# Xinglab/abPOA

Measured on AMD Instinct MI355X. Metric: read-sets/sec (consensus bit-exact) + DP Gcells/sec (roofline.dp_gcells_per_s), higher is better.
Workload: dtype int16

## Files before the change

### abpoa_amd/csrc/diag.h

```cpp
#pragma once
#include <stdint.h>

#if defined(__HIPCC__)
#define DIAG_HD __host__ __device__
#else
#define DIAG_HD
#endif

namespace abpoa_hip {

constexpr int DBG_NO_FAST_LOOPS = 64;
constexpr int DBG_KEEP_ROW_SLOTS = 128;
constexpr int DBG_WALK_REPORT = 256;
constexpr int DBG_WALK_GIVES_UP = 512;
constexpr int DBG_ONE_WAVE_BACKTRACK = 1024;
constexpr int DBG_CXX_TIGHT_LOOP = 2048;
constexpr int ABL_NO_ARENA_STORE = 1;
constexpr int ABL_FAST_NO_RING_STORE = 2,     ABL_GEN_FAKE_ARGMAX = 2;
constexpr int ABL_FAST_NO_ARGMAX = 4,         ABL_GEN_LITERAL_F_SCAN = 4;
constexpr int ABL_FAST_NO_F_CLOSED_FORM = 8,  ABL_GEN_NO_CHUNKS = 8;
constexpr int ABL_FAST_NO_GATHER = 16,        ABL_GEN_FAKE_GATHER = 16;
constexpr int ABL_FAST_NO_SLOW_F = 32,        ABL_GEN_NO_QUERY_PROFILE = 32;
constexpr int DBG_ABLATION_BITS = 63;
struct DbgBit { int value; const char *what; };
constexpr DbgBit DBG_BITS[] = {
    {DBG_ABLATION_BITS, "timing ablations of the row loops (1 .. 32: only in a `make prof` library, results wrong on purpose)"},
    {DBG_NO_FAST_LOOPS, "no fast row loops"}, {DBG_KEEP_ROW_SLOTS, "the tails keep the row loop's AlnOut.seg"}, {DBG_WALK_REPORT, "walk report in AlnOut.seg"},
    {DBG_WALK_GIVES_UP, "the direction-word walk gives up (NEED_SCORES)"}, {DBG_ONE_WAVE_BACKTRACK, "one wavefront per backtrack"},
    {DBG_CXX_TIGHT_LOOP, "the compiler's tight loop"},
};

#ifdef ABPOA_HIP_PROFILE
#define FSTAMP(I) { asm volatile("s_waitcnt lgkmcnt(0)" ::: "memory"); long long t_ = (long long)__builtin_amdgcn_s_memtime(); fseg[I] += t_ - fseg_last; fseg_last = t_; }
#else
#define FSTAMP(I)
#endif
#ifdef ABPOA_HIP_ASM_CENSUS
#define CENSUS_SLOT(I) ((I) == CEN_ONE_PRED ? CEN_CXX_TIGHT : (I))
#else
#define CENSUS_SLOT(I) (I)
#endif
#ifdef ABPOA_HIP_ROW_CENSUS
#define CENSUS_T0() const long long cen_t0 = (long long)__builtin_amdgcn_s_memtime();
#define CENSUS(I) { fseg[CENSUS_SLOT(I)] += census_pack(1, (long long)__builtin_amdgcn_s_memtime() - cen_t0); }
#else
#define CENSUS_T0()
#define CENSUS(I)
#endif
#ifdef ABPOA_HIP_WIDE_COUNTERS
#define WCOUNT(I) { fseg[I] += 1; }
#define WCOUNT_BODY(NCH) { fseg[WC_BODY] += wide_body_pack(1, 0, 0) + ((NCH) >= 9 ? (I16 ? wide_body_pack(0, 0, 1) : wide_body_pack(0, 1, 0)) : 0); }
#else
#define WCOUNT(I) {}
#define WCOUNT_BODY(NCH) {}
#endif
#ifdef ABPOA_HIP_ABLATE
#define ABL(BIT) (b.dbg & (BIT))
#else
#define ABL(BIT) false
#endif

constexpr int DIAG_SLOTS = 6;
// ... 27 lines not shown
```

### abpoa_amd/csrc/engine_options.cpp

```cpp
#include "engine_options.h"
#include "diag.h"
#include <atomic>
#include <cstdlib>
#include <cstring>
#include <mutex>
#include <string>

namespace abpoa_hip {
namespace {

struct Row { const char *name, *help; };
const std::string kDbgHelp = [] { std::string h = "D  bit mask handed to the kernels (DevBatch.dbg; diag.h):";
                                  for (const DbgBit &d : DBG_BITS) h += (&d == DBG_BITS ? " " : ", ") + std::to_string(d.value) + " " + d.what;
                                  return h; }();
const Row kTable[] = {
    {"ABPOA_GPU_DEVICES", "P  device ordinals abpoa_hip_msa_batch spreads its batches over: all | 0,1,... (default: the device of abpoa_hip_init)"},
    {"ABPOA_GPU_BATCHES_PER_DEVICE", "P  batches dealt per device queue [2]"},
    {"ABPOA_HIP_STRICT", "P  1: a call that would hand any read-set to the host driver fails with ABPOA_HIP_ESTRICT"},
    {"ABPOA_HIP_VERBOSE", "P  per-pass timings, residency and fallback reasons on stderr"},
    {"ABPOA_HIP_HOSTGRAPH", "T  1: the host driver for every job"},
    {"ABPOA_HIP_NO_DEVICE_STRAND", "T  1: -s jobs on the host driver"},
    {"ABPOA_HIP_NO_DEVICE_LOCAL", "T  1: local-mode jobs on the host driver"},
    {"ABPOA_HIP_NO_DEVICE_GENERAL", "T  1: general-kernel jobs on the host driver"},
    {"ABPOA_HIP_DEVICE_GENERAL", "T  1: the general kernel for every device-resident job"},
    {"ABPOA_HIP_LOCKSTEP", "T  1: one launch per phase and round also where the all-rounds kernel would run"},
    {"ABPOA_HIP_LATE_TAIL", "T  1: the helpers of the all-rounds kernel's backtrack start after the row loop, not under it"},
    {"ABPOA_HIP_NODIR", "T  1: score-record arenas instead of direction words"},
    {"ABPOA_HIP_DIR_WIDE", "T  1 / 0: direction words for wide-band alignments always / never (default: by residency and memory)"},
    {"ABPOA_HIP_NOFAST", "T  1: no fast row loops (general kernel)"},
    {"ABPOA_HIP_NOWIDE", "T  1: no wide row loop"},
    {"ABPOA_HIP_NOXL", "T  1: no long-read form of the wide row loop"},
    {"ABPOA_HIP_LOCAL_TEAM", "T  1 / 0: the four-wavefront local row loop always / never"},
    {"ABPOA_HIP_WIDE_LO", "T  smallest band half-width that takes the wide loop [40]"},
    {"ABPOA_HIP_RING_ROWS", "T  depth of the wide loop's score ring (4 | 8 | 16)"},
    {"ABPOA_HIP_EXTRA_ROUTE_MIN", "T  ragged sets with fewer extra columns keep the narrow loop"},
    {"ABPOA_HIP_NO_RAGGED_SPLIT", "T  1: read-sets with ragged read ends stay in the batch of the uniform ones (no all-rounds kernel for such a job)"},
    {"ABPOA_HIP_RAGGED_CONCURRENT", "T  1: the ragged batch of a mixed job runs on a second queue of the device beside the uniform batch (measured: see LOG.md)"},
    {"ABPOA_HIP_PASS_SETS", "T  read-sets per pass of the device-resident driver"},
    {"ABPOA_HIP_FIRST_PASS", "T  start the node-slot ladder (3x, 4.5x, 6x, 4096x) at its second / third / fourth pass: 1 / 2 / 3 (profiling runs of one step)"},
    {"ABPOA_HIP_NO_PASS_HINT", "T  1: always start the ladder at 3x"},
    {"ABPOA_HIP_GROUPS", "T  read-set groups of the host driver"},
    {"ABPOA_HIP_ARENA_PCT", "T  arena estimate in percent (overflow-retry tests)"},
    {"ABPOA_HIP_BT_BYTES", "T  LDS window of the tail kernel in bytes"},
    {"ABPOA_HIP_BT_WC", "T  columns per row of the tail's column-slice windows"},
    {"ABPOA_HIP_ORDER_LDS", "T  0: the row-order walk with global tables"},
    {"ABPOA_HIP_ORDER_CAP", "T  node capacity of the row-order walk's LDS tables"},
// ... 59 lines not shown
```

### abpoa_amd/csrc/rows_fast.h

```cpp
#pragma once
#include "dp_common.h"
#include "dir_plane.h"
#include "rows_tight_asm.h"
#include "wide_closed_forms.h"

namespace abpoa_hip {

template <typename T, int GAP> struct FastFmt { static constexpr int CW = GAP == 0 ? 2 : (GAP == 1 ? 4 : 8); };
static_assert(FastFmt<int, 0>::CW == record_values(ABPOA_HIP_LINEAR_GAP) && FastFmt<int, 1>::CW == record_values(ABPOA_HIP_AFFINE_GAP) && FastFmt<int, 2>::CW == record_values(ABPOA_HIP_CONVEX_GAP), "engine.h record_values");
template <typename T, int GAP> struct DirFmt {
    static constexpr int DB = GAP == 1 ? 2 : 4;
    static constexpr int UPV2 = Width<T>::PN * DB / 16;
    __device__ __host__ static constexpr int units(int nv) { return (nv * UPV2 + 1) >> 1; }
};
template <int GAP> __device__ __forceinline__ unsigned dir_word(unsigned kf, unsigned u1, unsigned u2, unsigned d1, unsigned d2) {
    static_assert(DIRA_DF1_SH - DIRA_UE1_SH == 3 && DIRC_UE2_SH - DIRC_UE1_SH == 3 && DIRC_DF2_SH - DIRC_DF1_SH == 3 && DIRC_DF1_SH - DIRC_UE1_SH == 8, "field layout of dir_plane.h");
    if (GAP == 1) return (((d1 << 3) | u1) << DIRA_UE1_SH) | kf;
    return (((((d2 << 3) | d1) << 8) | ((u2 << 3) | u1)) << DIRC_UE1_SH) | kf;
}
template <int GAP> __device__ __forceinline__ unsigned dir_pack(unsigned kM, unsigned kE1, unsigned kE2, unsigned u1, unsigned u2, unsigned d1, unsigned d2) {
    return dir_word<GAP>(GAP == 1 ? (kE1 << DIRA_KE1_SH) | kM : (((kE2 << 4) | kE1) << DIRC_KE1_SH) | kM, u1, u2, d1, d2);
}
__device__ __forceinline__ unsigned umin_(unsigned a, unsigned b) { return a < b ? a : b; }
template <typename T> __device__ __forceinline__ unsigned dir_literal(int Hm1, int Fm1, int F, int oe, int e) {
// ... 65 lines not shown
    int *fr = (int *)(lds_raw + ph_off + b.lds.fr_off);
    typedef __attribute__((address_space(3))) int lds_int_t;
    const int vslot = (int)(unsigned)(size_t)(lds_int_t *)fr + 4 * ((threadIdx.x & 63 & (RR - 1)) * (NPW * RCS) + 2);
    auto ring_at = [&](int slot_addr, int col_idx) __attribute__((always_inline)) { return (const int *)(lds_int_t *)(size_t)(unsigned)(slot_addr + 4 * col_idx); };
    int *s_mx = (int *)(lds_raw + (WIDEB ? b.lds.w_mx_off : b.lds.mx_off));
    auto qat = [&](int j) __attribute__((always_inline)) -> int {
        if constexpr (WIDEB) return ((int)s_query[j >> 1] >> ((j & 1) * 4)) & 15; else return (int)s_query[j];
    };
    const int infw = I16 ? (int)(((unsigned)inf & 0xffffu) | ((unsigned)inf << 16)) : inf;
    const int qlen_sn = qlen / PN;
    auto wr = [](int x) __attribute__((always_inline)) { return (int)(T)x; };

    const int idist = inj_dist<PN>(l);
    const int inj1 = idist >= 0 ? inf - idist * e1 : INT_MIN, inj2 = idist >= 0 ? inf - idist * e2 : INT_MIN;
    const int le1 = lane * e1, le2 = lane * e2;
    const int cf1 = oe1 - e1 + le1, cf2 = oe2 - e2 + le2;
    const long long lo_ll = (long long)(I16 ? INT16_MIN : INT32_MIN) + imax(oe1, oe2) + (long long)PN * imax(e1, e2);
    const int fast_lo = (int)lo_ll;
    const int kconst = I16 ? argmax_key16_const(PN, l, vvl) : 0;
    const int ktie = argmax_tie32(PN, l, vvl);

    { GLOBAL_AS const int32_t *g_mat = vgpr_ptr(b.mat); for (int i = lane; i < m * m1; i += 64) { const int bb = i / m1, qc = i - bb * m1; s_mx[i] = qc < m ? g_mat[bb * m + qc] : 0; } }
    for (int i = lane; i < RR * NPW * RCS; i += 64) { const int pl = (i / RCS) % NPW; fr[i] = (I16 && pl == 0) ? infw : ((EPACK && pl == 1) ? 0 : inf); }
    WG_SYNC();
    auto ring_put = [&](int slot, int x, int H, int E1, int E2) __attribute__((always_inline)) {
        int *q = fr + slot * (NPW * RCS) + 2 + x;
        if (I16) { q[0] = (int)(((unsigned)H & 0xffffu) | ((unsigned)E1 << 16)); if (GAP == 2) q[RCS] = E2; }
        else { q[0] = H; if (GAP != 0) q[RCS] = E1; if (GAP == 2) q[2 * RCS] = E2; }
    };

    const bool extend = sgpr(b.align_mode == ABPOA_HIP_EXTEND_MODE ? 1 : 0) != 0;
    int ex_best = inf, ex_i = 0, ex_j = 0, ex_rem = 0; bool zstop = false;
    const bool asm_tight_on = sgpr(!(b.dbg & DBG_CXX_TIGHT_LOOP) && RC == 128 && b.align_mode != ABPOA_HIP_EXTEND_MODE ? 1 : 0) != 0;
    int cur = 0, n_vec_lane = 0;
    const int cap_pn = (int)(d.plane_cap / PN > 0x7fffffffLL ? 0x7fffffffLL : d.plane_cap / PN);
    const int cap_turbo = cap_pn - (DIR ? dir_units(NV) + NV * CWR : NV * CW);
    const int remain_end = __builtin_amdgcn_readfirstlane(io.row_remain[gn - 1]);
    int vg_geo = 0, vg_mi = 0, vg_off = 0;
    int vg_vm = 0, rowmax = 0;
    {
        const int r = __builtin_amdgcn_readfirstlane(io.row_remain[0]) - remain_end - 1;
        const int dp_end0 = imin(qlen, imax(0, qlen - r) + w);
        const int end_sn0 = dp_end0 / PN, W0 = (end_sn0 + 1) * PN;
        if ((long long)W0 * CWR > d.plane_cap) { status = ABPOA_HIP_STATUS_OVERFLOW; cursor_out = 0; n_cells_out = 0; rows_done_out = 0; return; }
        const bool ring0 = W0 <= RC && !EPACK;
        T *H = io.planes;
        for (int i = lane; i < W0; i += 64) {
            int h, x1 = inf, x2 = inf, f1 = inf, f2 = inf;
            if (GAP == 0) h = wr(-e1 * i);
            else if (GAP == 1) { const int g = wr(-o1 - e1 * i); h = i == 0 ? 0 : g; x1 = i == 0 ? wr(-oe1) : inf; f1 = i == 0 ? inf : g; }
            else {
                const int g1 = wr(-o1 - e1 * i), g2 = wr(-o2 - e2 * i);
                h = i == 0 ? 0 : imax(g1, g2); x1 = i == 0 ? wr(-oe1) : inf; x2 = i == 0 ? wr(-oe2) : inf; f1 = i == 0 ? inf : g1; f2 = i == 0 ? inf : g2;
            }
            T *cellp = H + (long long)i * CWR;
            if constexpr (CPK) { cellp[0] = (T)h; cellp[1] = (T)(i == 0 ? (int)((unsigned)(h - x1) | ((unsigned)(h - x2) << 16)) : -1); }
            else if constexpr (CSP) { cellp[0] = (T)h; cellp[PL_E1] = (T)x1; if (GAP == 2) { cellp[PL_E2] = (T)x2; cellp[3] = (T)0; } }
            else if constexpr (GAP == 0) { cellp[0] = (T)h; cellp[1] = (T)0; }
            else {
                cellp[0] = (T)h; cellp[PL_E1] = (T)x1; cellp[PL_F1] = (T)f1;
                if (GAP == 2) { cellp[PL_E2] = (T)x2; cellp[PL_F2] = (T)f2; }
            }
            if (ring0) ring_put(0, i, h, x1, x2);
        }
        cur = (end_sn0 + 1) * CWR;
        if (lane == 0) { vg_geo = (end_sn0 << 12) | (ring0 ? GEO_RING : 0); vg_mi = 0; vg_off = DIR ? cur : 0; }
// ... 12 lines not shown
        MetaB q; const int np = a.pe - a.ps;
#pragma unroll
        for (int k = 0; k < NPM; ++k) q.p[k] = io.pred_row[a.ps + imin(k, imax(np - 1, 0))];
        return q;
    };
    MetaA a1 = load_a(0); MetaB b1 = load_b(a1); MetaA a2 = load_a(64);
    int tv_r1 = 0, tv_r2 = 0;
    int tv_meta = 0, tv_rterm = 0, tv_ps = 0, tv_p0 = 0, tv_p1 = 0, tv_p2 = 0, tv_p3 = 0;
    int tv_p4 = 0, tv_p5 = 0, tv_p6 = 0, tv_p7 = 0;
    int tv_tb = 0;
    auto switch_tile = [&](int t0) __attribute__((always_inline)) {
        const int myrow = t0 + lane, np = a1.pe - a1.ps;
        bool fastrow = np >= 1 && np <= 4 && myrow < gn - 1 && myrow >= 1;
#pragma unroll
        for (int k = 0; k < 4; ++k) { const int dk = myrow - b1.p[k]; fastrow = fastrow && dk >= 1 && dk < RR; }
        tv_meta = (a1.base & 0xff) | (imin(np, 255) << 8) | (fastrow ? (1 << 16) : 0);
        if (!WIDEB) {
            tv_meta |= ((fastrow && np <= 2 && RC <= 128) ? (1 << 17) : 0) | ((fastrow && np >= 3 && RC <= 128) ? (1 << 18) : 0);
            bool row8 = np >= 5 && np <= 8 && myrow < gn - 1 && myrow >= 1 && RC <= 128;
#pragma unroll
            for (int k = 0; k < NPM; ++k) { const int dk = myrow - b1.p[k]; row8 = row8 && dk >= 1 && dk < RR; }
            tv_meta |= row8 ? (1 << 20) : 0;
        }
        {
            bool widerow = np >= 1 && np <= 8 && myrow < gn - 1 && myrow >= 1;
#pragma unroll
            for (int k = 0; k < NPM; ++k) { const int dk = myrow - b1.p[k]; widerow = widerow && dk >= 1 && dk < 64; }
            tv_meta |= widerow ? (1 << 19) : 0;
        }
        if constexpr (DIR) {
            const bool sp = a1.sd >= RR;
            if (sp) { tv_meta |= 1 << 21; if (tv_meta & (1 << 17)) tv_meta = (tv_meta & ~(1 << 17)) | (1 << 22); }
        }
        tv_tb = ((myrow - b1.p[0]) & 0xff) | (((myrow - b1.p[1]) & 0xff) << 8) | (((a1.base & 0xff) * m1 * 4) << 16);
        tv_rterm = qlen - (a1.rem - remain_end - 1); tv_ps = a1.ps;
        tv_r1 = imin(gn, tv_rterm) - w; tv_r2 = tv_rterm + w;
        tv_p0 = b1.p[0]; tv_p1 = b1.p[1]; tv_p2 = b1.p[2]; tv_p3 = b1.p[3];
        tv_p4 = b1.p[4]; tv_p5 = b1.p[5]; tv_p6 = b1.p[6]; tv_p7 = b1.p[7];
        a1 = a2; b1 = load_b(a1); a2 = load_a(t0 + 128);
    };
    int qc_beg_sn = -1, qoff0 = 0, qoff1 = 0;
    auto geo_of = [&](int p, int row, int &geo, int &mi, int &off) __attribute__((always_inline)) {
        if (row - p < 64) { const int sl = p & 63; geo = __builtin_amdgcn_readlane(vg_geo, sl); mi = __builtin_amdgcn_readlane(vg_mi, sl); off = __builtin_amdgcn_readlane(vg_off, sl); }
        else {
            geo = __builtin_amdgcn_readfirstlane(gld_i32(io.g_bsn + p) | (gld_i32(io.g_esn + p) << 12)); mi = __builtin_amdgcn_readfirstlane(gld_i32(io.row_max_i + p));
            off = __builtin_amdgcn_readfirstlane((int)(uint32_t)(gld_i64(io.g_coff + p) / PN));
        }
    };
    int beg_sn = 0, end_sn = 0, off_pn = 0, max_pe = 0, rterm = 0, base = 0, np = 0;
    bool to_ring = false;
    unsigned am_key = 0; int am_val = INT_MIN, am_v = 0, am_isend = 0; bool am_any = false;

    auto set_band = [&](auto pin, int mn_mi, int mx_mi, int min_pb) __attribute__((always_inline)) {
        auto S = [](int x) __attribute__((always_inline)) { if constexpr (decltype(pin)::value) return sgpr(x); else return x; };
        const int left = S(imin(gn, mn_mi + 1)), right = S(decltype(pin)::value ? mx_mi + 1 : imax(0, mx_mi + 1));
        const int lo = S(imin(left, rterm) - w), hi = S(imax(right, rterm) + w);
        const int beg = S(imax(0, lo)), end = S(imin(qlen, hi));
        beg_sn = imax((int)((unsigned)beg / PN), min_pb); end_sn = (int)((unsigned)end / PN);
    };
    auto refresh_qc = [&]() __attribute__((always_inline)) {
        if (beg_sn != qc_beg_sn) {
            qc_beg_sn = beg_sn;
            const int c0 = beg_sn * PN + lane, c1 = c0 + 64;
            qoff0 = (c0 >= 1 && c0 <= qlen) ? qat(c0 - 1) : m; qoff1 = (c1 >= 1 && c1 <= qlen) ? qat(c1 - 1) : m;
        }
    };
// ... 1062 lines not shown
```

### abpoa_amd/csrc/rows_tight_asm.h

```cpp
#pragma once
#define TA_SDWA0 " dst_sel:DWORD dst_unused:UNUSED_PAD src0_sel:WORD_0 src1_sel:DWORD\n\t"
#define TA_SDWA_S1W0 " dst_sel:DWORD dst_unused:UNUSED_PAD src0_sel:DWORD src1_sel:WORD_0\n\t"
#define TA_SDWA_S1W1 " dst_sel:DWORD dst_unused:UNUSED_PAD src0_sel:DWORD src1_sel:WORD_1\n\t"
#define TA_SDWA_S0W1 " dst_sel:DWORD dst_unused:UNUSED_PAD src0_sel:WORD_1 src1_sel:DWORD\n\t"
#define TA_DPP(CTRL) " " CTRL " bank_mask:0xf\n\t"
#define vQA "v104"
#define vCOL "v105"
#define vX "v106"
#define vQ "v107"
#define vR0 "v108"
#define vR1 "v109"
#define vR01 "v[108:109]"
#define vKC "v110"
#define vH "v111"
#define vHSE "v112"
#define vAK "v113"
#define vS1 "v114"
#define vG "v115"
#define vF "v115"
#define vQD "v116"
#define vRO "v117"
#define vHO "v118"
#define vT2A "v119"
#define vEN "v120"
// ... 3 lines not shown
#define vD "v123"
#define vKF "v124"
#define vWD "v124"
#define vX1 "v125"
#define vB0 "v126"
#define vB1 "v127"
#define vB01 "v[126:127]"
#define vMV "v100"
#define vE1 "v101"
#define vMV2 "v102"
#define vE12 "v103"
#define vT "v106"
#define vP "v125"
#define vFS "v126"
#define vSH "v127"
#define vKM "v92"
#define vKE "v93"
#define vX2 "v94"
#define vX3 "v95"
#define vC0 "v96"
#define vC1 "v97"
#define vC01 "v[96:97]"
#define vD0 "v98"
#define vD1 "v99"
#define vD01 "v[98:99]"

#define TA_BAND_BEG                                                                                          \
    "s_min_i32 %[sA], %[sA], %[sRT]\n\t"  "s_max_i32 %[sA], %[sA], 0\n\t"       "s_lshr_b32 %[sA], %[sA], 4\n\t"
#define TA_BAND_END                                                                                          \
    "s_max_i32 %[sB], %[sB], %[sR2]\n\t"  "s_min_i32 %[sB], %[sB], %[qlen]\n\t" "s_lshr_b32 %[sESN], %[sB], 4\n\t"
#define TA_QCACHE(LBL)                                                                                       \
    "s_cmp_lg_u32 %[sBSN], %[qcb]\n\t"     "s_cbranch_scc1 L_ref" LBL "_%=\n\t"                              \
    "L_refd" LBL "_%=:\n\t"
#define TA_CHECKS(SLOWLBL)                                                                                   \
    "s_sub_i32 %[sNV1], %[sESN], %[sBSN]\n\t"                                                                \
    "s_cmp_gt_u32 %[sNV1], 3\n\t"          "s_cbranch_scc1 L_dec_%=\n\t"                                     \
    "s_cmp_gt_i32 %[sESN], %[sPE0]\n\t"    "s_cbranch_scc1 " SLOWLBL "_%=\n\t"
#define TA_RINGCHK                                                                                           \
    "s_bitcmp0_b32 %[sG0], 24\n\t"         "s_cbranch_scc1 L_dec_%=\n\t"
#define TA_SLOW_ENTRY(SLOWLBL)                                                                               \
    TA_ALIGN SLOWLBL "_%=:\n\t"                                                                                       \
    "s_add_i32 %[sA], %[sPE0], 1\n\t"      "s_cmp_lg_u32 %[sESN], %[sA]\n\t"      "s_cbranch_scc1 L_dec_%=\n\t" \
    "s_cmp_gt_u32 %[sBSN], %[sPE0]\n\t"    "s_cbranch_scc1 L_dec_%=\n\t"
#define TA_S_YES(x) x
#define TA_S_NO(x) ""
#define TA_REFRESH(LBL)                                                                                      \
    "L_ref" LBL "_%=:\n\t"                                                                                   \
    "s_mov_b32 %[qcb], %[sBSN]\n\t"        "s_lshl_b32 %[sA], %[sBSN], 4\n\t"     "s_add_i32 %[sA], %[sA], -1\n\t"      \
    "v_add_u32 " vX ", %[sA], %[lane]\n\t" "v_cmp_gt_u32 vcc, %[qlen], " vX "\n\t" "v_add_u32 " vQ ", %[qb], " vX "\n\t" \
    "ds_read_u8 " vQ ", " vQ "\n\t"                                                                          \
    "v_add_u32 " vX ", 64, " vX "\n\t"     "v_cmp_gt_u32_e64 %[msk], %[qlen], " vX "\n\t" "v_add_u32 " vG ", %[qb], " vX "\n\t" \
    "ds_read_u8 " vG ", " vG "\n\t"        "v_mov_b32 " vX ", %[m]\n\t"                                      \
    "s_waitcnt lgkmcnt(0)\n\t"                                                                               \
    "v_cndmask_b32 %[qoff0], " vX ", " vQ ", vcc\n\t"   "v_cndmask_b32_e64 %[qoff1], " vX ", " vG ", %[msk]\n\t"  \
    "v_lshl_add_u32 " vQA ", %[qoff0], 2, %[mxb]\n\t"                                                        \
    "s_branch L_refd" LBL "_%=\n\t"
#define TA_READS                                                                                             \
    "s_lshl_b32 %[sC0], %[sBSN], 4\n\t"    "v_add_u32 " vCOL ", %[sC0], %[lane]\n\t"                         \
    "s_ashr_i32 %[sA], %[sTB], 16\n\t"     "v_add_u32 " vX ", %[sA], " vQA "\n\t"    "ds_read_b32 " vQ ", " vX "\n\t"   \
    "s_lshl_b32 %[sA], %[sPB0], 4\n\t"     "v_xad_u32 " vX ", %[sA], -1, " vCOL "\n\t"  "v_med3_i32 " vX ", " vX ", -2, %[rc]\n\t" \
    "v_lshl_add_u32 " vX ", " vX ", 2, %[sSL0]\n\t"   "ds_read2_b32 " vR01 ", " vX " offset1:1\n\t"
#define TA_MASKS                                                                                             \
    "v_cmp_ge_u32_e64 %[inb], %[sNV1], %[vvl]\n\t"                                                               \
    "v_cmp_eq_u32 vcc, %[sNV1], %[vvl]\n\t"      "v_cndmask_b32 " vKC ", %[kN], %[kE], vcc\n\t"              \
    "v_cmp_ge_i32_e64 %[amok], %[qlen], " vCOL "\n\t"  "s_and_b64 %[amok], %[amok], %[inb]\n\t"
#define TA_SCAN                                                                                              \
    "v_add_u32 " vG ", " vH ", %[le1]\n\t"                                                                  \
    "v_lshl_add_u32 " vAK ", " vHSE ", 16, " vKC "\n\t"   "v_cndmask_b32_e64 " vAK ", 0, " vAK ", %[amok]\n\t" \
    "v_subrev_u32 " vS1 ", %[e1], " vH "\n\t"                                                               \
    "v_mov_b32_dpp " vS1 ", " vG " wave_shr:1 row_mask:0xf bank_mask:0xf\n\t"                                \
    "v_max_u32_dpp " vAK ", " vAK ", " vAK TA_DPP("row_shr:1 row_mask:0xf")                                  \
    "v_readlane_b32 %[sP0], %[vslot], %[row]\n\t"                                                            \
    "v_max_i32_dpp " vS1 ", " vS1 ", " vS1 TA_DPP("row_shr:1 row_mask:0xf")                                  \
    "v_max_u32_dpp " vAK ", " vAK ", " vAK TA_DPP("row_shr:2 row_mask:0xf")                                  \
    "s_lshl_b32 %[sM0], %[cur], 5\n\t"                                                                       \
    "v_max_i32_dpp " vS1 ", " vS1 ", " vS1 TA_DPP("row_shr:2 row_mask:0xf")                                  \
// ... 29 lines not shown
    TA_SLOW_STEP("3", "16", "row_shr:8")
#define TA_SLOW_F                                                                                            \
    "v_cmp_eq_u32 vcc, %[sNV1], %[vvl]\n\t"     "v_cndmask_b32 " vF ", " vF ", " vFS ", vcc\n\t"
#define TA_SLOW_LIT                                                                                          \
    "v_mov_b32_dpp " vP ", " vHO " wave_shr:1 row_mask:0xf bank_mask:0xf\n\t"                                \
    "v_mov_b32_dpp " vSH ", " vF " wave_shr:1 row_mask:0xf bank_mask:0xf\n\t"                                \
    "v_subrev_u32 " vP ", %[oe1], " vP "\n\t"   "v_bfe_i32 " vP ", " vP ", 0, 16\n\t"   "v_cmp_eq_i32_e64 %[msk], " vP ", " vF "\n\t" \
    "v_subrev_u32 " vSH ", %[e1], " vSH "\n\t"  "v_bfe_i32 " vSH ", " vSH ", 0, 16\n\t" "v_cmp_eq_i32 vcc, " vSH ", " vF "\n\t" \
    "v_cndmask_b32_e64 " vSH ", 3, 2, vcc\n\t"  "v_cndmask_b32_e64 " vSH ", " vSH ", 1, %[msk]\n\t"          \
    "v_cmp_le_u32 vcc, %[sNV1], %[vvl]\n\t"     "v_cndmask_b32 " vSH ", 0, " vSH ", vcc\n\t"
#define TA_HEF(EN_INSTR, S)                                                                                  \
    "v_sub_u32 " vF ", " vS1 ", %[cf1]\n\t"     "v_max_i32 " vF ", " vF ", %[inj1]\n\t"                      \
    S(TA_SLOW_F)                                                                                             \
    "v_max_i32 " vHO ", " vHSE ", " vF "\n\t"   "v_subrev_u32 " vT2A ", %[oe1], " vHO "\n\t"                 \
    EN_INSTR                                                                                                 \
    "v_max_i32 " vEN ", " vEN ", " vT2A "\n\t"                                                               \
    "v_cmp_lt_i32 vcc, " vHSE ", " vF "\n\t"    "v_cndmask_b32 " vE ", " vEN ", %[infv], vcc\n\t"            \
    "v_sub_u32 " vU ", " vEN ", " vT2A "\n\t"   "v_sub_u32 " vD ", " vHO ", " vF "\n\t"     "v_min_u32 " vD ", 7, " vD "\n\t" \
    "v_perm_b32 " vHE ", " vE ", " vHO ", %[perm]\n\t"                                                       \
    S(TA_SLOW_LIT)
#define TA_TAIL(S)                                                                                           \
    "v_lshl_or_b32 " vU ", " vD ", 3, " vU "\n\t"   "v_lshl_or_b32 " vWD ", " vU ", 8, " vKF "\n\t"           \
    S("v_lshl_or_b32 " vWD ", " vSH ", 14, " vWD "\n\t")                                                     \
    "global_store_short " vRO ", " vWD ", %[planes]\n\t"                                                     \
    "v_cndmask_b32_e64 " vHE ", %[infwv], " vHE ", %[inb]\n\t"                                                   \
    "ds_write2st64_b32 " vQD ", " vHE ", %[infwv] offset1:1\n\t"                                             \
    "v_readlane_b32 %[sA], " vAK ", 63\n\t"                                                                  \
    "s_bitset1_b32 %[sB], 24\n\t"                                                                            \
    "v_writelane_b32 %[geo], %[sB], m0\n\t"     "v_writelane_b32 %[off], %[cur], m0\n\t"                     \
    "s_and_b32 %[sM0], %[sA], 63\n\t"           "s_add_i32 %[sM0], %[sM0], %[sC0]\n\t"                       \
    "s_cmp_gt_u32 %[sA], %[infk]\n\t"           "s_cselect_b32 %[sA], %[sM0], -1\n\t"       \
    "v_writelane_b32 %[mi], %[sA], m0\n\t"                                                                   \
    "s_add_i32 %[cur], %[cur], %[sNV1]\n\t"     "s_add_i32 %[cur], %[cur], 1\n\t"                            \
    "s_add_i32 %[row], %[row], 1\n\t"           "s_cmp_lt_i32 %[row], %[rhi]\n\t"     "s_cbranch_scc1 L_row_%=\n\t"

#define TA_IF4_YES(x) x
#define TA_IF4_NO(x) ""
#define TA_FOLD(LANE, SL, PB, PE)                                                                            \
    "v_readlane_b32 %[sM1], %[mi], " LANE "\n\t"  "v_readlane_b32 %[sG1], %[geo], " LANE "\n\t"  "v_readlane_b32 " SL ", %[vslot], " LANE "\n\t" \
    "s_min_i32 %[sA], %[sA], %[sM1]\n\t"          "s_max_i32 %[sB], %[sB], %[sM1]\n\t"           "s_and_b32 %[sG0], %[sG0], %[sG1]\n\t" \
    "s_and_b32 " PB ", %[sG1], 0xfff\n\t"         "s_bfe_u32 " PE ", %[sG1], 0xc000c\n\t"
#define TA_READK(X, PAIR, SL, PB, PE)                                                                        \
    "s_lshl_b32 %[sA], " PB ", 4\n\t"             "v_subrev_u32 " X ", %[sA], " vCOL "\n\t"                  \
    "v_add_u32 " vT ", -1, " X "\n\t"             "v_med3_i32 " vT ", " vT ", -2, %[rc]\n\t"                 \
    "v_lshl_add_u32 " vT ", " vT ", 2, " SL "\n\t"  "ds_read2_b32 " PAIR ", " vT " offset1:1\n\t"            \
    "s_sub_i32 " PE ", " PE ", " PB "\n\t"        "s_lshl_b32 " PE ", " PE ", 4\n\t"             "s_add_i32 " PE ", " PE ", 16\n\t"
#define TA_MERGE(KIDX, W0, W1, X, PE)                                                                        \
    "v_max_i32_sdwa " vT ", " vMV ", sext(" W0 ")" TA_SDWA_S1W0                                              \
    "v_cmp_lt_i32 vcc, " vMV ", " vT "\n\t"                                                                  \
    "s_add_i32 %[sA], " PE ", 16\n\t"             "v_cmp_gt_u32_e64 %[msk], %[sA], " X "\n\t"    "s_and_b64 vcc, vcc, %[msk]\n\t" \
    "v_cndmask_b32_e64 " vKM ", " vKM ", " KIDX ", vcc\n\t"   "v_cndmask_b32_e64 " vMV ", " vMV ", " vT ", %[msk]\n\t" \
    "v_max_i32_sdwa " vT ", " vE1 ", sext(" W1 ")" TA_SDWA_S1W1                                              \
    "v_cmp_lt_i32 vcc, " vE1 ", " vT "\n\t"                                                                  \
    "v_cmp_gt_u32_e64 %[msk], " PE ", " X "\n\t"  "s_and_b64 vcc, vcc, %[msk]\n\t"                           \
    "v_cndmask_b32_e64 " vKE ", " vKE ", " KIDX ", vcc\n\t"   "v_cndmask_b32_e64 " vE1 ", " vE1 ", " vT ", %[msk]\n\t"
#define TA_MULTI_POST(IF4, S)                                                                                \
    TA_RINGCHK                                                                                               \
    TA_MASKS                                                                                                 \
    "v_mov_b32 " vKM ", 1\n\t"                    "v_mov_b32 " vKE ", 1\n\t"                                 \
    "s_waitcnt lgkmcnt(0)\n\t"                                                                               \
    "v_bfe_i32 " vMV ", " vR0 ", 0, 16\n\t"       "v_ashrrev_i32 " vE1 ", 16, " vR1 "\n\t"                   \
    TA_MERGE("2", vB0, vB1, vX1, "%[sPE1]")                                                                  \
    TA_MERGE("3", vC0, vC1, vX2, "%[sPE2]")                                                                  \
    IF4(TA_MERGE("4", vD0, vD1, vX3, "%[sPE3]"))                                                             \
    "v_add_u32 " vH ", " vMV ", " vQ "\n\t"                                                                  \
    "v_min_i32 " vT ", " vH ", " vE1 "\n\t"                                                                  \
    "v_cmp_gt_i32 vcc, %[fastlo], " vT "\n\t"     "s_and_b64 %[msk], %[inb], vcc\n\t"   "s_cbranch_scc1 L_x2_%=\n\t"  \
    "v_max_i32 " vHSE ", " vH ", " vE1 "\n\t"                                                                \
    TA_SCAN                                                                                                  \
    S(TA_SLOW_A)                                                                                             \
    TA_HEF("v_subrev_u32 " vEN ", %[e1], " vE1 "\n\t", S)                                                    \
    "v_cmp_eq_u32 vcc, " vH ", " vHO "\n\t"       "v_cndmask_b32 " vKF ", 0, " vKM ", vcc\n\t"               \
    "v_lshl_or_b32 " vKF ", " vKE ", 4, " vKF "\n\t"                                                         \
    TA_TAIL(S)                                                                                               \
    "s_branch L_end_%=\n\t"
#define TA_MULTI(IF4, LBL)                                                                                   \
    "s_mov_b32 %[sA], %[sM0]\n\t"                 "s_mov_b32 %[sB], %[sM0]\n\t"                              \
    "s_and_b32 %[sPB0], %[sG0], 0xfff\n\t"        "s_bfe_u32 %[sPE0], %[sG0], 0xc000c\n\t"                   \
    TA_FOLD("%[sP1]", "%[sSL1]", "%[sPB1]", "%[sPE1]")                                                       \
    TA_FOLD("%[sP2]", "%[sSL2]", "%[sPB2]", "%[sPE2]")                                                       \
    IF4(TA_FOLD("%[sP3]", "%[sSL3]", "%[sPB3]", "%[sPE3]"))                                                  \
    "s_add_i32 %[sA], %[sA], %[c1]\n\t"               "s_add_i32 %[sB], %[sB], %[c2]\n\t"                            \
    TA_BAND_BEG                                                                                              \
    "s_min_u32 %[sESN], %[sPB0], %[sPB1]\n\t"     "s_min_u32 %[sESN], %[sESN], %[sPB2]\n\t"   IF4("s_min_u32 %[sESN], %[sESN], %[sPB3]\n\t") \
    "s_max_u32 %[sBSN], %[sA], %[sESN]\n\t"                                                                  \
    TA_QCACHE(LBL)                                                                                           \
    TA_READS                                                                                                 \
    "s_max_u32 %[sPE0], %[sPE0], %[sPE1]\n\t"     "s_max_u32 %[sPE0], %[sPE0], %[sPE2]\n\t" IF4("s_max_u32 %[sPE0], %[sPE0], %[sPE3]\n\t") \
    TA_READK(vX1, vB01, "%[sSL1]", "%[sPB1]", "%[sPE1]")                                                     \
    TA_READK(vX2, vC01, "%[sSL2]", "%[sPB2]", "%[sPE2]")                                                     \
    IF4(TA_READK(vX3, vD01, "%[sSL3]", "%[sPB3]", "%[sPE3]"))                                                \
    TA_BAND_END                                                                                              \
    TA_CHECKS("L_s" LBL)                                                                                     \
    TA_MULTI_POST(IF4, TA_S_NO)                                                                              \
    TA_SLOW_ENTRY("L_s" LBL)                                                                                 \
    TA_MULTI_POST(IF4, TA_S_YES)

#define TA_ONE_POST(S)                                                                                       \
    TA_RINGCHK                                                                                               \
    TA_MASKS                                                                                                 \
    "s_waitcnt lgkmcnt(0)\n\t"                                                                               \
    "v_add_u32_sdwa " vH ", sext(" vR0 "), " vQ TA_SDWA0                                                     \
    "v_min_i32_sdwa " vT ", " vH ", sext(" vR1 ")" TA_SDWA_S1W1                                              \
    "v_cmp_gt_i32 vcc, %[fastlo], " vT "\n\t"   "s_and_b64 %[msk], %[inb], vcc\n\t"   "s_cbranch_scc1 L_x2_%=\n\t"  \
    "v_max_i32_sdwa " vHSE ", " vH ", sext(" vR1 ")" TA_SDWA_S1W1                                            \
    TA_SCAN                                                                                                  \
    S(TA_SLOW_A)                                                                                             \
    TA_HEF("v_sub_u32_sdwa " vEN ", sext(" vR1 "), %[e1]" TA_SDWA_S0W1, S)                                   \
    "v_cmp_eq_u32 vcc, " vH ", " vHO "\n\t"     "v_cndmask_b32_e64 " vKF ", 16, 17, vcc\n\t"                 \
    TA_TAIL(S)                                                                                               \
    "s_branch L_end_%=\n\t"
#define TA_TWO_POST(S)                                                                                       \
    TA_RINGCHK                                                                                               \
    TA_MASKS                                                                                                 \
    "s_waitcnt lgkmcnt(0)\n\t"                                                                               \
    "v_bfe_i32 " vMV ", " vR0 ", 0, 16\n\t"     "v_ashrrev_i32 " vE1 ", 16, " vR1 "\n\t"                     \
    "v_max_i32_sdwa " vT ", " vMV ", sext(" vB0 ")" TA_SDWA_S1W0                                             \
    "v_cmp_gt_u32 vcc, %[sP1], " vX1 "\n\t"     "v_cndmask_b32 " vMV2 ", " vMV ", " vT ", vcc\n\t"           \
    "v_max_i32_sdwa " vT ", " vE1 ", sext(" vB1 ")" TA_SDWA_S1W1                                             \
    "v_cmp_gt_u32 vcc, %[sM1], " vX1 "\n\t"     "v_cndmask_b32 " vE12 ", " vE1 ", " vT ", vcc\n\t"           \
    "v_add_u32 " vH ", " vMV2 ", " vQ "\n\t"                                                                 \
    "v_min_i32 " vT ", " vH ", " vE12 "\n\t"                                                                 \
    "v_cmp_gt_i32 vcc, %[fastlo], " vT "\n\t"   "s_and_b64 %[msk], %[inb], vcc\n\t"   "s_cbranch_scc1 L_x2_%=\n\t"  \
    "v_max_i32 " vHSE ", " vH ", " vE12 "\n\t"                                                               \
    TA_SCAN                                                                                                  \
    S(TA_SLOW_A)                                                                                             \
    TA_HEF("v_subrev_u32 " vEN ", %[e1], " vE12 "\n\t", S)                                                   \
    "v_cmp_ne_u32 vcc, " vMV2 ", " vMV "\n\t"   "v_cndmask_b32_e64 " vKF ", 1, 2, vcc\n\t"                   \
    "v_cmp_eq_u32 vcc, " vH ", " vHO "\n\t"     "v_cndmask_b32 " vKF ", 0, " vKF ", vcc\n\t"                 \
    "v_cmp_ne_u32 vcc, " vE12 ", " vE1 "\n\t"   "v_cndmask_b32_e64 " vX ", 16, 32, vcc\n\t"                  \
    "v_or_b32 " vKF ", " vKF ", " vX "\n\t"                                                                  \
    TA_TAIL(S)                                                                                               \
    "s_branch L_end_%=\n\t"

#ifndef ABPOA_HIP_ASM_ALIGN
#define ABPOA_HIP_ASM_ALIGN 6
#endif
#define TA_STR2(x) #x
#define TA_STR(x) TA_STR2(x)
#define TA_ALIGN ".p2align " TA_STR(ABPOA_HIP_ASM_ALIGN) "\n\t"
#define TA_LOOP_HEAD "s_branch L_row_%=\n\t" TA_ALIGN
#define TIGHT_ASM_I16_AFFINE_DIR                                                                             \
    "v_lshl_add_u32 " vQA ", %[qoff0], 2, %[mxb]\n\t"                                                        \
    "s_mov_b32 %[code], 3\n\t"                                                                               \
    TA_LOOP_HEAD                                                                                             \
    "L_row_%=:\n\t"                                                                                          \
    "v_readlane_b32 %[sM], %[tvmeta], %[row]\n\t"   "v_readlane_b32 %[sTB], %[tvtb], %[row]\n\t"   "v_readlane_b32 %[sRT], %[tvr1], %[row]\n\t" \
    "v_readlane_b32 %[sR2], %[tvr2], %[row]\n\t"                                                            \
    "s_and_b32 m0, %[row], 63\n\t"                                                                           \
    "s_and_b32 %[sA], %[sTB], 0xff\n\t"         "s_sub_i32 %[sP0], %[row], %[sA]\n\t"                        \
    "v_readlane_b32 %[sM0], %[mi], %[sP0]\n\t"  "v_readlane_b32 %[sG0], %[geo], %[sP0]\n\t"   "v_readlane_b32 %[sSL0], %[vslot], %[sP0]\n\t" \
    "s_bitcmp1_b32 %[sM], 17\n\t"               "s_cbranch_scc0 L_n17_%=\n\t"                                \
    "s_bitcmp1_b32 %[sM], 9\n\t"                "s_cbranch_scc1 L_two_%=\n\t"                                \
                                                                       \
    "s_add_i32 %[sA], %[sM0], %[c1]\n\t"        "s_add_i32 %[sB], %[sM0], %[c2]\n\t"                                 \
    TA_BAND_BEG                                                                                              \
    "s_and_b32 %[sPB0], %[sG0], 0xfff\n\t"      "s_max_u32 %[sBSN], %[sA], %[sPB0]\n\t"                      \
    TA_QCACHE("1")                                                                                           \
    TA_READS                                                                                                 \
    TA_BAND_END                                                                                              \
    "s_bfe_u32 %[sPE0], %[sG0], 0xc000c\n\t"                                                                 \
    TA_CHECKS("L_s1")                                                                                        \
    TA_ONE_POST(TA_S_NO)                                                                                     \
    TA_SLOW_ENTRY("L_s1")                                                                                    \
    TA_ONE_POST(TA_S_YES)                                                                                    \
                                                                      \
    TA_ALIGN "L_two_%=:\n\t"                                                                                          \
    "s_bfe_u32 %[sA], %[sTB], 0x80008\n\t"      "s_sub_i32 %[sP1], %[row], %[sA]\n\t"                        \
    "v_readlane_b32 %[sM1], %[mi], %[sP1]\n\t"  "v_readlane_b32 %[sG1], %[geo], %[sP1]\n\t"   "v_readlane_b32 %[sSL1], %[vslot], %[sP1]\n\t" \
    "s_min_i32 %[sA], %[sM0], %[sM1]\n\t"       "s_max_i32 %[sB], %[sM0], %[sM1]\n\t"                        \
    "s_add_i32 %[sA], %[sA], %[c1]\n\t"             "s_add_i32 %[sB], %[sB], %[c2]\n\t"                              \
    TA_BAND_BEG                                                                                              \
    "s_and_b32 %[sPB0], %[sG0], 0xfff\n\t"      "s_and_b32 %[sPB1], %[sG1], 0xfff\n\t"                       \
    "s_min_u32 %[sESN], %[sPB0], %[sPB1]\n\t"   "s_max_u32 %[sBSN], %[sA], %[sESN]\n\t"                      \
    TA_QCACHE("2")                                                                                           \
    TA_READS                                                                                                 \
    "s_lshl_b32 %[sA], %[sPB1], 4\n\t"          "v_subrev_u32 " vX1 ", %[sA], " vCOL "\n\t"                  \
    "v_add_u32 " vX ", -1, " vX1 "\n\t"         "v_med3_i32 " vX ", " vX ", -2, %[rc]\n\t"                   \
    "v_lshl_add_u32 " vX ", " vX ", 2, %[sSL1]\n\t"   "ds_read2_b32 " vB01 ", " vX " offset1:1\n\t"           \
    TA_BAND_END                                                                                              \
    "s_bfe_u32 %[sPE0], %[sG0], 0xc000c\n\t"    "s_bfe_u32 %[sPE1], %[sG1], 0xc000c\n\t"                     \
    "s_sub_i32 %[sM1], %[sPE1], %[sPB1]\n\t"    "s_lshl_b32 %[sM1], %[sM1], 4\n\t"                           \
    "s_add_i32 %[sM1], %[sM1], 16\n\t"          "s_add_i32 %[sP1], %[sM1], 16\n\t"                           \
    "s_max_u32 %[sPE0], %[sPE0], %[sPE1]\n\t"   "s_and_b32 %[sG0], %[sG0], %[sG1]\n\t"                       \
    TA_CHECKS("L_s2")                                                                                        \
    TA_TWO_POST(TA_S_NO)                                                                                     \
    TA_SLOW_ENTRY("L_s2")                                                                                    \
    TA_TWO_POST(TA_S_YES)                                                                                    \
                                                             \
    TA_ALIGN "L_n17_%=:\n\t"                                                                                          \
    "s_bitcmp1_b32 %[sM], 18\n\t"               "s_cbranch_scc0 L_x0_%=\n\t"                                 \
    "s_bitcmp1_b32 %[sM], 21\n\t"               "s_cbranch_scc1 L_x0_%=\n\t"                                 \
    "v_readlane_b32 %[sP2], %[tvp2], %[row]\n\t"  "v_readlane_b32 %[sP3], %[tvp3], %[row]\n\t"               \
    "s_bfe_u32 %[sA], %[sTB], 0x80008\n\t"      "s_sub_i32 %[sP1], %[row], %[sA]\n\t"                        \
    "s_bitcmp1_b32 %[sM], 10\n\t"               "s_cbranch_scc1 L_four_%=\n\t"                               \
    TA_MULTI(TA_IF4_NO, "3")                                                                                 \
    TA_ALIGN "L_four_%=:\n\t"                                                                                         \
    TA_MULTI(TA_IF4_YES, "4")                                                                                \
                                                                           \
    TA_REFRESH("1")                                                                                          \
    TA_REFRESH("2")                                                                                          \
    TA_REFRESH("3")                                                                                          \
    TA_REFRESH("4")                                                                                          \
    "L_dec_%=:\n\t"                                                                                          \
    "s_waitcnt lgkmcnt(0)\n\t"                   \
    "s_mov_b32 %[code], 2\n\t"                                                                               \
    "s_cmp_gt_u32 %[sNV1], 3\n\t"               "s_cbranch_scc1 L_end_%=\n\t"                                \
    "s_cmp_gt_i32 %[sBSN], %[sPE0]\n\t"         "s_cbranch_scc1 L_end_%=\n\t"                                \
    "s_bitcmp0_b32 %[sG0], 24\n\t"              "s_cbranch_scc1 L_end_%=\n\t"                                \
    "s_mov_b32 %[code], 1\n\t"                  "s_branch L_end_%=\n\t"                                      \
    "L_x0_%=:\n\t"  "s_mov_b32 %[code], 0\n\t"  "s_branch L_end_%=\n\t"                                      \
    "L_x2_%=:\n\t"  "s_mov_b32 %[code], 2\n\t"                                                               \
    "L_end_%=:\n\t"
```

Baseline: 20250.

## Forward previous row's H/E registers to chained single-predecessor rows in asm loop

Adds a chain path to the hand-written tight assembly row loop. When a row's only predecessor is the immediately preceding row, a new meta bit (23) is set. For such rows the loop reuses the previous row's H values, shifted one lane with DPP, along with its E values held in registers, so the predecessor row is not reloaded from the LDS score ring. A separate decline label handles rows that must fall back, and a debug bit can turn the path off. This adds branch complexity and code size in the inner loop, and correctness depends on the forwarded registers exactly matching the ring contents.

```diff
diff --git a/abpoa_amd/csrc/diag.h b/abpoa_amd/csrc/diag.h
--- a/abpoa_amd/csrc/diag.h
+++ b/abpoa_amd/csrc/diag.h
@@ -15,6 +15,7 @@
 constexpr int DBG_WALK_GIVES_UP = 512;
 constexpr int DBG_ONE_WAVE_BACKTRACK = 1024;
 constexpr int DBG_CXX_TIGHT_LOOP = 2048;
+constexpr int DBG_NO_CHAIN_FORWARD = 4096;
 constexpr int ABL_NO_ARENA_STORE = 1;
 constexpr int ABL_FAST_NO_RING_STORE = 2,     ABL_GEN_FAKE_ARGMAX = 2;
 constexpr int ABL_FAST_NO_ARGMAX = 4,         ABL_GEN_LITERAL_F_SCAN = 4;
@@ -28,6 +29,9 @@
     {DBG_NO_FAST_LOOPS, "no fast row loops"}, {DBG_KEEP_ROW_SLOTS, "the tails keep the row loop's AlnOut.seg"}, {DBG_WALK_REPORT, "walk report in AlnOut.seg"},
     {DBG_WALK_GIVES_UP, "the direction-word walk gives up (NEED_SCORES)"}, {DBG_ONE_WAVE_BACKTRACK, "one wavefront per backtrack"},
     {DBG_CXX_TIGHT_LOOP, "the compiler's tight loop"},
+};
+constexpr DbgBit DBG_AB_BITS[] = {
+    {DBG_NO_CHAIN_FORWARD, "the assembly loop forwards nothing from row to row"},
 };
 
 #ifdef ABPOA_HIP_PROFILE
diff --git a/abpoa_amd/csrc/engine_options.cpp b/abpoa_amd/csrc/engine_options.cpp
--- a/abpoa_amd/csrc/engine_options.cpp
+++ b/abpoa_amd/csrc/engine_options.cpp
@@ -12,6 +12,7 @@
 struct Row { const char *name, *help; };
 const std::string kDbgHelp = [] { std::string h = "D  bit mask handed to the kernels (DevBatch.dbg; diag.h):";
                                   for (const DbgBit &d : DBG_BITS) h += (&d == DBG_BITS ? " " : ", ") + std::to_string(d.value) + " " + d.what;
+                                  for (const DbgBit &d : DBG_AB_BITS) h += ", " + std::to_string(d.value) + " " + d.what;
                                   return h; }();
 const Row kTable[] = {
     {"ABPOA_GPU_DEVICES", "P  device ordinals abpoa_hip_msa_batch spreads its batches over: all | 0,1,... (default: the device of abpoa_hip_init)"},
diff --git a/abpoa_amd/csrc/rows_fast.h b/abpoa_amd/csrc/rows_fast.h
--- a/abpoa_amd/csrc/rows_fast.h
+++ b/abpoa_amd/csrc/rows_fast.h
@@ -121,6 +121,7 @@
     const bool extend = sgpr(b.align_mode == ABPOA_HIP_EXTEND_MODE ? 1 : 0) != 0;
     int ex_best = inf, ex_i = 0, ex_j = 0, ex_rem = 0; bool zstop = false;
     const bool asm_tight_on = sgpr(!(b.dbg & DBG_CXX_TIGHT_LOOP) && RC == 128 && b.align_mode != ABPOA_HIP_EXTEND_MODE ? 1 : 0) != 0;
+    const bool chain_on = sgpr(!(b.dbg & DBG_NO_CHAIN_FORWARD) ? 1 : 0) != 0;
     int cur = 0, n_vec_lane = 0;
     const int cap_pn = (int)(d.plane_cap / PN > 0x7fffffffLL ? 0x7fffffffLL : d.plane_cap / PN);
     const int cap_turbo = cap_pn - (DIR ? dir_units(NV) + NV * CWR : NV * CW);
@@ -199,6 +200,7 @@
             const bool sp = a1.sd >= RR;
             if (sp) { tv_meta |= 1 << 21; if (tv_meta & (1 << 17)) tv_meta = (tv_meta & ~(1 << 17)) | (1 << 22); }
         }
+        if (!WIDEB && chain_on && (tv_meta & (1 << 17)) && np == 1 && myrow - b1.p[0] == 1) tv_meta |= 1 << 23;
         tv_tb = ((myrow - b1.p[0]) & 0xff) | (((myrow - b1.p[1]) & 0xff) << 8) | (((a1.base & 0xff) * m1 * 4) << 16);
         tv_rterm = qlen - (a1.rem - remain_end - 1); tv_ps = a1.ps;
         tv_r1 = imin(gn, tv_rterm) - w; tv_r2 = tv_rterm + w;
diff --git a/abpoa_amd/csrc/rows_tight_asm.h b/abpoa_amd/csrc/rows_tight_asm.h
--- a/abpoa_amd/csrc/rows_tight_asm.h
+++ b/abpoa_amd/csrc/rows_tight_asm.h
@@ -59,16 +59,16 @@
 #define TA_QCACHE(LBL)                                                                                       \
     "s_cmp_lg_u32 %[sBSN], %[qcb]\n\t"     "s_cbranch_scc1 L_ref" LBL "_%=\n\t"                              \
     "L_refd" LBL "_%=:\n\t"
-#define TA_CHECKS(SLOWLBL)                                                                                   \
+#define TA_CHECKS(SLOWLBL, DEC)                                                                              \
     "s_sub_i32 %[sNV1], %[sESN], %[sBSN]\n\t"                                                                \
-    "s_cmp_gt_u32 %[sNV1], 3\n\t"          "s_cbranch_scc1 L_dec_%=\n\t"                                     \
+    "s_cmp_gt_u32 %[sNV1], 3\n\t"          "s_cbranch_scc1 " DEC "_%=\n\t"                                   \
     "s_cmp_gt_i32 %[sESN], %[sPE0]\n\t"    "s_cbranch_scc1 " SLOWLBL "_%=\n\t"
 #define TA_RINGCHK                                                                                           \
     "s_bitcmp0_b32 %[sG0], 24\n\t"         "s_cbranch_scc1 L_dec_%=\n\t"
-#define TA_SLOW_ENTRY(SLOWLBL)                                                                               \
+#define TA_SLOW_ENTRY(SLOWLBL, DEC)                                                                          \
     TA_ALIGN SLOWLBL "_%=:\n\t"                                                                                       \
-    "s_add_i32 %[sA], %[sPE0], 1\n\t"      "s_cmp_lg_u32 %[sESN], %[sA]\n\t"      "s_cbranch_scc1 L_dec_%=\n\t" \
-    "s_cmp_gt_u32 %[sBSN], %[sPE0]\n\t"    "s_cbranch_scc1 L_dec_%=\n\t"
+    "s_add_i32 %[sA], %[sPE0], 1\n\t"      "s_cmp_lg_u32 %[sESN], %[sA]\n\t"      "s_cbranch_scc1 " DEC "_%=\n\t" \
+    "s_cmp_gt_u32 %[sBSN], %[sPE0]\n\t"    "s_cbranch_scc1 " DEC "_%=\n\t"
 #define TA_S_YES(x) x
 #define TA_S_NO(x) ""
 #define TA_REFRESH(LBL)                                                                                      \
@@ -164,7 +164,7 @@
     "s_cmp_gt_u32 %[sA], %[infk]\n\t"           "s_cselect_b32 %[sA], %[sM0], -1\n\t"       \
     "v_writelane_b32 %[mi], %[sA], m0\n\t"                                                                   \
     "s_add_i32 %[cur], %[cur], %[sNV1]\n\t"     "s_add_i32 %[cur], %[cur], 1\n\t"                            \
-    "s_add_i32 %[row], %[row], 1\n\t"           "s_cmp_lt_i32 %[row], %[rhi]\n\t"     "s_cbranch_scc1 L_row_%=\n\t"
+    "s_add_i32 %[row], %[row], 1\n\t"           "s_cmp_lt_i32 %[row], %[rhi]\n\t"     "s_cbranch_scc1 L_chain_%=\n\t"
 
 #define TA_IF4_YES(x) x
 #define TA_IF4_NO(x) ""
@@ -223,25 +223,56 @@
     TA_READK(vX2, vC01, "%[sSL2]", "%[sPB2]", "%[sPE2]")                                                     \
     IF4(TA_READK(vX3, vD01, "%[sSL3]", "%[sPB3]", "%[sPE3]"))                                                \
     TA_BAND_END                                                                                              \
-    TA_CHECKS("L_s" LBL)                                                                                     \
+    TA_CHECKS("L_s" LBL, "L_dec")                                                                                     \
     TA_MULTI_POST(IF4, TA_S_NO)                                                                              \
-    TA_SLOW_ENTRY("L_s" LBL)                                                                                 \
+    TA_SLOW_ENTRY("L_s" LBL, "L_dec")                                                                                 \
     TA_MULTI_POST(IF4, TA_S_YES)
 
+#define TA_ONE_CELLS(S, R1)                                                                                  \
+    "s_waitcnt lgkmcnt(0)\n\t"                                                                               \
+    "v_add_u32_sdwa " vH ", sext(" vR0 "), " vQ TA_SDWA0                                                     \
+    "v_min_i32_sdwa " vT ", " vH ", sext(" R1 ")" TA_SDWA_S1W1                                               \
+    "v_cmp_gt_i32 vcc, %[fastlo], " vT "\n\t"   "s_and_b64 %[msk], %[inb], vcc\n\t"   "s_cbranch_scc1 L_x2_%=\n\t"  \
+    "v_max_i32_sdwa " vHSE ", " vH ", sext(" R1 ")" TA_SDWA_S1W1                                             \
+    TA_SCAN                                                                                                  \
+    S(TA_SLOW_A)                                                                                             \
+    TA_HEF("v_sub_u32_sdwa " vEN ", sext(" R1 "), %[e1]" TA_SDWA_S0W1, S)                                    \
+    "v_cmp_eq_u32 vcc, " vH ", " vHO "\n\t"     "v_cndmask_b32_e64 " vKF ", 16, 17, vcc\n\t"                 \
+    TA_TAIL(S)                                                                                               \
+    "s_branch L_end_%=\n\t"
 #define TA_ONE_POST(S)                                                                                       \
     TA_RINGCHK                                                                                               \
     TA_MASKS                                                                                                 \
-    "s_waitcnt lgkmcnt(0)\n\t"                                                                               \
-    "v_add_u32_sdwa " vH ", sext(" vR0 "), " vQ TA_SDWA0                                                     \
-    "v_min_i32_sdwa " vT ", " vH ", sext(" vR1 ")" TA_SDWA_S1W1                                              \
-    "v_cmp_gt_i32 vcc, %[fastlo], " vT "\n\t"   "s_and_b64 %[msk], %[inb], vcc\n\t"   "s_cbranch_scc1 L_x2_%=\n\t"  \
-    "v_max_i32_sdwa " vHSE ", " vH ", sext(" vR1 ")" TA_SDWA_S1W1                                            \
-    TA_SCAN                                                                                                  \
-    S(TA_SLOW_A)                                                                                             \
-    TA_HEF("v_sub_u32_sdwa " vEN ", sext(" vR1 "), %[e1]" TA_SDWA_S0W1, S)                                   \
-    "v_cmp_eq_u32 vcc, " vH ", " vHO "\n\t"     "v_cndmask_b32_e64 " vKF ", 16, 17, vcc\n\t"                 \
-    TA_TAIL(S)                                                                                               \
-    "s_branch L_end_%=\n\t"
+    TA_ONE_CELLS(S, vR1)
+
+#define TA_CHAIN_BIT "23"
+#define TA_CHAIN_CELLS(S)                                                                                    \
+    "v_mov_b32 " vR0 ", %[infwv]\n\t"                                                                        \
+    "v_mov_b32_dpp " vR0 ", " vHE " wave_shr:1 row_mask:0xf bank_mask:0xf\n\t"                               \
+    TA_ONE_CELLS(S, vHE)
+#define TA_CHAIN_POST(S)                                                                                     \
+    TA_MASKS                                                                                                 \
+    TA_CHAIN_CELLS(S)
+#define TA_CHAIN_BODY                                                                                        \
+    "s_add_i32 %[sB], %[sA], %[c2]\n\t"         "s_add_i32 %[sA], %[sA], %[c1]\n\t"                          \
+    TA_BAND_BEG                                                                                              \
+    "s_max_u32 %[sA], %[sA], %[sBSN]\n\t"       "s_cmp_lg_u32 %[sA], %[sBSN]\n\t"     "s_cbranch_scc1 L_cmv_%=\n\t" \
+    "s_ashr_i32 %[sA], %[sTB], 16\n\t"          "v_add_u32 " vX ", %[sA], " vQA "\n\t"   "ds_read_b32 " vQ ", " vX "\n\t" \
+    "s_mov_b32 %[sPE0], %[sESN]\n\t"                                                                         \
+    TA_BAND_END                                                                                              \
+    TA_CHECKS("L_sc", "L_decc")                                                                              \
+    TA_CHAIN_POST(TA_S_NO)                                                                                   \
+    TA_SLOW_ENTRY("L_sc", "L_decc")                                                                          \
+    TA_CHAIN_POST(TA_S_YES)
+#define TA_CHAIN_MOVED                                                                                       \
+    "L_cmv_%=:\n\t"                                                                                          \
+    "s_mov_b32 %[sPB0], %[sBSN]\n\t"            "s_mov_b32 %[sBSN], %[sA]\n\t"        "s_add_i32 %[sP0], %[row], -1\n\t" \
+    "v_readlane_b32 %[sG0], %[geo], %[sP0]\n\t" "v_readlane_b32 %[sSL0], %[vslot], %[sP0]\n\t"               \
+    "s_branch L_one_%=\n\t"
+#define TA_ROW_WORDS                                                                                         \
+    "v_readlane_b32 %[sM], %[tvmeta], %[row]\n\t"   "v_readlane_b32 %[sTB], %[tvtb], %[row]\n\t"   "v_readlane_b32 %[sRT], %[tvr1], %[row]\n\t" \
+    "v_readlane_b32 %[sR2], %[tvr2], %[row]\n\t"                                                            \
+    "s_and_b32 m0, %[row], 63\n\t"
 #define TA_TWO_POST(S)                                                                                       \
     TA_RINGCHK                                                                                               \
     TA_MASKS                                                                                                 \
@@ -272,14 +303,21 @@
 #define TA_STR(x) TA_STR2(x)
 #define TA_ALIGN ".p2align " TA_STR(ABPOA_HIP_ASM_ALIGN) "\n\t"
 #define TA_LOOP_HEAD "s_branch L_row_%=\n\t" TA_ALIGN
+#ifndef ABPOA_HIP_ASM_CHAIN_BRANCH
+#define TA_CHAIN_PLACED "s_cbranch_scc0 L_gen_%=\n\t" TA_CHAIN_BODY TA_ALIGN "L_row_%=:\n\t" TA_ROW_WORDS "L_gen_%=:\n\t"
+#define TA_CHAIN_OUT_OF_LINE TA_CHAIN_MOVED
+#else
+#define TA_CHAIN_PLACED "s_cbranch_scc1 L_ch_%=\n\t" "L_gen_%=:\n\t"
+#define TA_CHAIN_OUT_OF_LINE "L_row_%=:\n\t" TA_ROW_WORDS "s_branch L_gen_%=\n\t" TA_ALIGN "L_ch_%=:\n\t" TA_CHAIN_BODY TA_CHAIN_MOVED
+#endif
 #define TIGHT_ASM_I16_AFFINE_DIR                                                                             \
     "v_lshl_add_u32 " vQA ", %[qoff0], 2, %[mxb]\n\t"                                                        \
     "s_mov_b32 %[code], 3\n\t"                                                                               \
     TA_LOOP_HEAD                                                                                             \
-    "L_row_%=:\n\t"                                                                                          \
-    "v_readlane_b32 %[sM], %[tvmeta], %[row]\n\t"   "v_readlane_b32 %[sTB], %[tvtb], %[row]\n\t"   "v_readlane_b32 %[sRT], %[tvr1], %[row]\n\t" \
-    "v_readlane_b32 %[sR2], %[tvr2], %[row]\n\t"                                                            \
-    "s_and_b32 m0, %[row], 63\n\t"                                                                           \
+    "L_chain_%=:\n\t"                                                                                        \
+    TA_ROW_WORDS                                                                                             \
+    "s_bitcmp1_b32 %[sM], " TA_CHAIN_BIT "\n\t"                                                              \
+    TA_CHAIN_PLACED                                                                                          \
     "s_and_b32 %[sA], %[sTB], 0xff\n\t"         "s_sub_i32 %[sP0], %[row], %[sA]\n\t"                        \
     "v_readlane_b32 %[sM0], %[mi], %[sP0]\n\t"  "v_readlane_b32 %[sG0], %[geo], %[sP0]\n\t"   "v_readlane_b32 %[sSL0], %[vslot], %[sP0]\n\t" \
     "s_bitcmp1_b32 %[sM], 17\n\t"               "s_cbranch_scc0 L_n17_%=\n\t"                                \
@@ -288,13 +326,14 @@
     "s_add_i32 %[sA], %[sM0], %[c1]\n\t"        "s_add_i32 %[sB], %[sM0], %[c2]\n\t"                                 \
     TA_BAND_BEG                                                                                              \
     "s_and_b32 %[sPB0], %[sG0], 0xfff\n\t"      "s_max_u32 %[sBSN], %[sA], %[sPB0]\n\t"                      \
+    "L_one_%=:\n\t"                                                                                          \
     TA_QCACHE("1")                                                                                           \
     TA_READS                                                                                                 \
     TA_BAND_END                                                                                              \
     "s_bfe_u32 %[sPE0], %[sG0], 0xc000c\n\t"                                                                 \
-    TA_CHECKS("L_s1")                                                                                        \
+    TA_CHECKS("L_s1", "L_dec")                                                                                        \
     TA_ONE_POST(TA_S_NO)                                                                                     \
-    TA_SLOW_ENTRY("L_s1")                                                                                    \
+    TA_SLOW_ENTRY("L_s1", "L_dec")                                                                                    \
     TA_ONE_POST(TA_S_YES)                                                                                    \
                                                                       \
     TA_ALIGN "L_two_%=:\n\t"                                                                                          \
@@ -315,9 +354,9 @@
     "s_sub_i32 %[sM1], %[sPE1], %[sPB1]\n\t"    "s_lshl_b32 %[sM1], %[sM1], 4\n\t"                           \
     "s_add_i32 %[sM1], %[sM1], 16\n\t"          "s_add_i32 %[sP1], %[sM1], 16\n\t"                           \
     "s_max_u32 %[sPE0], %[sPE0], %[sPE1]\n\t"   "s_and_b32 %[sG0], %[sG0], %[sG1]\n\t"                       \
-    TA_CHECKS("L_s2")                                                                                        \
+    TA_CHECKS("L_s2", "L_dec")                                                                                        \
     TA_TWO_POST(TA_S_NO)                                                                                     \
-    TA_SLOW_ENTRY("L_s2")                                                                                    \
+    TA_SLOW_ENTRY("L_s2", "L_dec")                                                                                    \
     TA_TWO_POST(TA_S_YES)                                                                                    \
                                                              \
     TA_ALIGN "L_n17_%=:\n\t"                                                                                          \
@@ -334,6 +373,13 @@
     TA_REFRESH("2")                                                                                          \
     TA_REFRESH("3")                                                                                          \
     TA_REFRESH("4")                                                                                          \
+    TA_CHAIN_OUT_OF_LINE                                                                                     \
+    "L_decc_%=:\n\t"                                \
+    "s_waitcnt lgkmcnt(0)\n\t"                                                                               \
+    "s_mov_b32 %[code], 2\n\t"                                                                               \
+    "s_cmp_gt_u32 %[sNV1], 3\n\t"               "s_cbranch_scc1 L_end_%=\n\t"                                \
+    "s_cmp_gt_i32 %[sBSN], %[sPE0]\n\t"         "s_cbranch_scc1 L_end_%=\n\t"                                \
+    "s_mov_b32 %[code], 1\n\t"                  "s_branch L_end_%=\n\t"                                      \
     "L_dec_%=:\n\t"                                                                                          \
     "s_waitcnt lgkmcnt(0)\n\t"                   \
     "s_mov_b32 %[code], 2\n\t"                                                                               \
```

Result: no change. 20320, median of 6 (+0.3%).
